# EdwardLiuyc/StaticMapping

Measured on NVIDIA H100. Metric: scan-pair alignments/sec (120k->500k pts, 30 ICP iters), higher is better.
Workload: dtype f64

## Files before the change

### include/sm_b200_debug.h

```cpp
#ifndef SM_B200_DEBUG_H_
#define SM_B200_DEBUG_H_

#include <stdint.h>

#ifdef __cplusplus
extern "C" {
#endif

int sm_debug_solve6(int device, const double* A_36, const double* b_6, double* x_6, int32_t* path);

int sm_debug_solve6_host(const double* A_36, const double* b_6, double* x_6, int32_t* path);

typedef int (*sm_debug_fdf)(const double* x_6, double* f, double* g_6, void* user);
int sm_debug_bfgs_minimize(sm_debug_fdf fn, void* user, double* x_6_inout, double grad_tol,
                           int32_t max_iterations, int32_t* iterations, int32_t* evaluations, int32_t* status);

int sm_debug_knn1_batched(int device, const double* target_3xn, int64_t n_target, const double* query_3xn,
                          int64_t n_query, double epsilon, int bucket_size, int32_t queries_per_cta,
                          int32_t* ids, double* dists2);

int sm_debug_ndt_host(int32_t op, const double* in, double* out);

int sm_debug_icp_host(int32_t op, const double* in, int64_t n, double* out);

typedef int (*sm_debug_ndt_eval)(const double* T_4x4, const double* p_6, double* sums_44, void* user);
int sm_debug_ndt_newton(sm_debug_ndt_eval fn, void* user, const double* guess_4x4, int32_t n_source, float resolution,
                        double step_size, double outlier_ratio, double transformation_epsilon, int32_t max_iterations,
                        double* final_4x4, int32_t* iterations, int32_t* evaluations, double* score);

typedef int (*sm_debug_gicp_correspond)(const double* transformation_4x4, const double* R_9, int32_t* m, void* user);
typedef int (*sm_debug_gicp_cost)(const double* T_4x4, double* S_13, void* user);
int sm_debug_gicp_outer(sm_debug_gicp_correspond correspond, sm_debug_gicp_cost cost, void* user,
                        const double* guess_4x4, double* final_4x4, int32_t* iterations, int32_t* bfgs_evaluations);

// ... 25 lines not shown
```

### staticmapping_b200/_lib.py

```python
from __future__ import annotations

import ctypes as C
import os

_HERE = os.path.dirname(os.path.abspath(__file__))
LIB_PATH = os.environ.get("SM_B200_LIB") or os.path.join(_HERE, "libsm_b200.so")


class AlignInfo(C.Structure):
    _fields_ = [("iterations", C.c_int32), ("status", C.c_int32), ("solve_path", C.c_int32),
                ("reserved", C.c_int32), ("kept", C.c_int64), ("limit", C.c_double),
                ("ms_upload", C.c_float), ("ms_prologue", C.c_float),
                ("ms_iterations", C.c_float), ("kernel_launches", C.c_int32),
                ("ms_knn", C.c_float), ("ms_accum", C.c_float), ("ms_finish", C.c_float),
                ("profiled_iterations", C.c_int32), ("evaluations", C.c_int32),
                ("trans_probability", C.c_double), ("mean_neighbors", C.c_double),
                ("aux", C.c_double * 4)]


class Pair(C.Structure):
    _fields_ = [("source", C.c_void_p), ("n_source", C.c_int64), ("target", C.c_void_p),
                ("target_normals", C.c_void_p), ("n_target", C.c_int64), ("guess", C.c_void_p),
                ("on_device", C.c_int32), ("reserved", C.c_int32)]

# ... 42 lines not shown
    "sm_debug_bfgs_minimize": (C.c_int, [_VP, _VP, _VP, C.c_double, C.c_int32, _VP, _VP, _VP]),
    "sm_debug_ndt_newton": (C.c_int, [_VP, _VP, _VP, C.c_int32, C.c_float, C.c_double, C.c_double, C.c_double, C.c_int32,
                                      _VP, _VP, _VP, _VP]),
    "sm_debug_normals_leaf": (C.c_int, [_VP, C.c_int32, _VP, _VP, _VP]),
    "sm_debug_voxel_index": (C.c_int, [C.c_int32, _VP, C.c_float, C.c_int32, _VP]),
    "sm_debug_gicp_point": (C.c_int, [C.c_int32, _VP, _VP]),
    "sm_debug_gicp_outer": (C.c_int, [_VP, _VP, _VP, _VP, _VP, _VP, _VP]),
    "sm_debug_gicp_host": (C.c_int, [C.c_int32, _VP, _VP]),
    "sm_debug_motion_host": (C.c_int, [_VP, C.c_int64, _DP, _VP]),
    "sm_debug_inner_compensation_host": (C.c_int, [_DP, _VP, _VP, _VP, C.c_int64, _VP, _VP]),
    "sm_debug_icp_host": (C.c_int, [C.c_int32, _VP, C.c_int64, _VP]),
    "sm_debug_ndt_leaf": (C.c_int, [_VP, C.c_int32, C.c_int32, C.c_double, _VP, _VP, _VP, _VP, _VP]),
    "sm_debug_ndt_term": (C.c_int, [_VP, C.c_double, C.c_float, C.c_int32, _VP, _VP, _VP, _VP, _VP]),
    "sm_debug_ndt_host": (C.c_int, [C.c_int32, _VP, _VP]),
    "sm_debug_knn1_batched": (C.c_int, [C.c_int, _VP, C.c_int64, _VP, C.c_int64, C.c_double, C.c_int, C.c_int32, _VP, _VP]),
    "sm_device_count": (C.c_int, []),
    "sm_version": (C.c_char_p, []),
}


def lib():
    global _lib
    if _lib is None:
        if not os.path.exists(LIB_PATH):
            raise RuntimeError(
                f"{LIB_PATH} not found: build it with `python -c 'import __graft_entry__ as g; "
                "g.build()'` (nvcc, sm_90a).  staticmapping_b200 has no CPU fallback.")
        _lib = C.CDLL(LIB_PATH)
        for name, (res, args) in SIGNATURES.items():
            fn = getattr(_lib, name)
# ... 4 lines not shown
```

### staticmapping_b200/csrc/icp.cu

```cuda
#include "common.cuh"
#include "kernels.h"
#include "icp_dev.cuh"
#include "knn_smem.cuh"
#include "linalg_dev.cuh"
#include "motion_dev.cuh"

#include <nvtx3/nvToolsExt.h>

namespace smb {
using namespace dev;
namespace {

__global__ void __launch_bounds__(256)
mean_partial_kernel(const double* __restrict__ raw, int64_t stride, int n,
                    double* __restrict__ partials) {
  __shared__ double sm[3][8];
  double s[3] = {0.0, 0.0, 0.0};
  const int base = blockIdx.x * 1024;
  for (int r = 0; r < 4; ++r) {
    const int i = base + r * 256 + threadIdx.x;
    if (i < n) { s[0] += raw[i]; s[1] += raw[stride + i]; s[2] += raw[2 * stride + i]; }
  }
  for (int d = 0; d < 3; ++d) {
    double v = s[d];
// ... 49 lines not shown
  st->hist_len = 1; st->iteration = 0; st->done = 0; st->status = 0; st->solve_path = 0;
  st->final_score = 0.0; st->limit = 0.0; st->kept = 0;
}

__device__ __forceinline__ uint32_t spread10(uint32_t v) {
  v &= 1023u;
  v = (v | (v << 16)) & 0x030000ffu;
  v = (v | (v << 8)) & 0x0300f00fu;
  v = (v | (v << 4)) & 0x030c30c3u;
  v = (v | (v << 2)) & 0x09249249u;
  return v;
}

__global__ void apply_g0_kernel(const double* __restrict__ in, double* __restrict__ out,
                                int64_t stride, int n, const IcpState* __restrict__ st,
                                uint64_t* __restrict__ keys, uint32_t* __restrict__ vals) {
  const int i = blockIdx.x * blockDim.x + threadIdx.x;
  if (i >= n) return;
  double px, py, pz;
  transform_point(st->G0, in[i], in[stride + i], in[2 * stride + i], px, py, pz);
  out[i] = px; out[stride + i] = py; out[2 * stride + i] = pz;
  const uint32_t ix = (uint32_t)(int)floor(px * 4.0), iy = (uint32_t)(int)floor(py * 4.0),
                 iz = (uint32_t)(int)floor(pz * 4.0);
  keys[i] = (uint64_t)(spread10(ix) | (spread10(iy) << 1) | (spread10(iz) << 2));
  vals[i] = (uint32_t)i;
}

__global__ void gather_source_kernel(const double* __restrict__ in, double* __restrict__ out,
                                     int64_t stride, int n, const uint32_t* __restrict__ perm) {
  const int i = blockIdx.x * blockDim.x + threadIdx.x;
  if (i >= n) return;
  const uint32_t s = perm[i];
  out[i] = in[s]; out[stride + i] = in[stride + s]; out[2 * stride + i] = in[2 * stride + s];
// ... 16 lines not shown
__global__ void __launch_bounds__(kKnnCtaThreads, SMB_KNN_MIN_CTAS)
icp_knn_kernel(IcpBuffers b, IcpParams p, int per_cta, const double* __restrict__ deskewed) {
  extern __shared__ __align__(128) unsigned char knn_smem[];
  if (b.state->done) return;
  uint64_t* bar; double* T;
  const SmemTree tree = stage_tree(b.kc, knn_smem, &bar, &T);
  if (threadIdx.x < 16) T[threadIdx.x] = b.state->T_iter[threadIdx.x];
  __syncthreads();
  const int begin = blockIdx.x * per_cta, end = min(begin + per_cta, p.n_source);
  int i = begin + threadIdx.x;
  double px = 0.0, py = 0.0, pz = 0.0;
  if (i < end) load_query<kComp>(b, T, deskewed, i, px, py, pz);
  mbar_wait(bar, 0);
  while (i < end) {
    int slot; double d2;
    knn1_smem<kAllSmem>(tree, px, py, pz, p.max_error2, slot, d2);
    b.slot[i] = slot;
    b.d2[i] = d2;
    if (finite_d2(d2)) atomicAdd(&b.hist[dist_bin(d2)], 1u);
    i += kKnnCtaThreads;
    if (i < end) load_query<kComp>(b, T, deskewed, i, px, py, pz);
  }
}

template <bool kAllSmem, bool kComp>
__global__ void __launch_bounds__(kKnnCtaThreads, SMB_KNN_MIN_CTAS)
icp_knn_batch_kernel(IcpBuffers b, IcpParams p, int per_cta, const double* __restrict__ deskewed) {
  extern __shared__ __align__(128) unsigned char knn_smem[];
  if (b.state->done) return;
  uint64_t* bar; double* T;
  const SmemTree tree = stage_tree(b.kc, knn_smem, &bar, &T);
  if (threadIdx.x < 16) T[threadIdx.x] = b.state->T_iter[threadIdx.x];
  __syncthreads();
  const int begin = blockIdx.x * per_cta, end = min(begin + per_cta, p.n_source);
  mbar_wait(bar, 0);
  knn_batch_cta<kAllSmem>(
      tree, begin, end, per_cta, p.max_error2, b.knn_items,
      [&](int i, double& x, double& y, double& z) { load_query<kComp>(b, T, deskewed, i, x, y, z); },
      [&](int i, int best, double head) { b.slot[i] = best; b.d2[i] = head; },
      [&](int i, double& head, int& best) { head = __ldcg(b.d2 + i); best = __ldcg(b.slot + i); },
      [&](int i, int slot, double d2) {
        b.slot[i] = slot;
        b.d2[i] = d2;
        if (finite_d2(d2)) atomicAdd(&b.hist[dist_bin(d2)], 1u);
      });
}

template <bool kComp>
__global__ void __launch_bounds__(kAccThreads)
icp_accum_kernel(IcpBuffers b, IcpParams p, const double* __restrict__ deskewed) {
  __shared__ uint32_t warp_tot[8];
  __shared__ BinSel sel_sm;
// ... 74 lines not shown
      const int64_t dst = tile0 + off + __popc(m[r] & ((1u << lane) - 1u));
      b.cand_key[dst] = (unsigned long long)__double_as_longlong(d2[r]);
      double2* o = reinterpret_cast<double2*>(b.cand_terms + 8 * dst);
      o[0] = make_double2(F[r][0], F[r][1]); o[1] = make_double2(F[r][2], F[r][3]);
      o[2] = make_double2(F[r][4], F[r][5]); o[3] = make_double2(dot[r], sq[r]);
    }
    base += tot;
  }
  if (threadIdx.x == 0) b.cand_cnt[blockIdx.x] = base;
  block_reduce_sums<kAccThreads>(acc, red, b.partials + (int64_t)blockIdx.x * 32);
}

template <bool kAllSmem>
__global__ void __launch_bounds__(kKnnCtaThreads)
knn_query_kernel(KdCompact kc, const double* __restrict__ query, int64_t qstride, int nq,
                 double max_error2, int per_cta, int32_t* __restrict__ ids, double* __restrict__ d2) {
  extern __shared__ __align__(128) unsigned char knn_smem[];
  uint64_t* bar; double* extra;
  const SmemTree tree = stage_tree(kc, knn_smem, &bar, &extra);
  const int begin = blockIdx.x * per_cta, end = min(begin + per_cta, nq);
  mbar_wait(bar, 0);
  for (int i = begin + threadIdx.x; i < end; i += kKnnCtaThreads) {
    int slot; double d;
    knn1_smem<kAllSmem>(tree, query[i], query[qstride + i], query[2 * qstride + i], max_error2, slot, d);
    ids[i] = slot >= 0 ? kc.pid[slot] : -1;
    d2[i] = d;
  }
}


template <bool kAllSmem>
__global__ void __launch_bounds__(kKnnCtaThreads, SMB_KNN_MIN_CTAS)
knn_query_batch_kernel(KdCompact kc, const double* __restrict__ query, int64_t qstride, int nq,
                       double max_error2, int per_cta, int32_t* __restrict__ ids, double* __restrict__ d2,
                       int4* __restrict__ items) {
  extern __shared__ __align__(128) unsigned char knn_smem[];
  uint64_t* bar; double* extra;
  const SmemTree tree = stage_tree(kc, knn_smem, &bar, &extra);
  const int begin = blockIdx.x * per_cta, end = min(begin + per_cta, nq);
  mbar_wait(bar, 0);
  knn_batch_cta<kAllSmem>(
      tree, begin, end, per_cta, max_error2, items,
      [&](int i, double& x, double& y, double& z) { x = query[i]; y = query[qstride + i]; z = query[2 * qstride + i]; },
      [&](int i, int best, double head) { ids[i] = best; d2[i] = head; },
      [&](int i, double& head, int& best) { head = __ldcg(d2 + i); best = __ldcg(ids + i); },
      [&](int i, int slot, double d) { ids[i] = slot >= 0 ? kc.pid[slot] : -1; d2[i] = d; });
}

}

int icp_accum_blocks(int n_source) { return ceil_div(n_source, kAccTile); }

static void knn_geometry(int nq, int queries_per_cta, int* grid, int* per_cta) {
  int per = queries_per_cta > 0 ? queries_per_cta : kKnnCtaThreads;
  per = ((per + kKnnCtaThreads - 1) / kKnnCtaThreads) * kKnnCtaThreads;
  *per_cta = per;
  *grid = ceil_div(nq, per);
}

int knn_query(const KdCompact& kc, const double* query, int64_t qstride, int nq, double max_error2,
              int32_t* ids, double* d2, cudaStream_t stream, int queries_per_cta, int4* items) {
  if (nq <= 0) return 0;
  int grid, per;
  knn_geometry(nq, queries_per_cta, &grid, &per);
  const size_t smem = knn_smem_bytes(kc.levels);
  const bool all = kc.levels <= kKnnSmemLevels;
  if (per > kKnnCtaThreads) {
    if (!items) return -1;
    if (all) knn_query_batch_kernel<true><<<grid, kKnnCtaThreads, smem, stream>>>(kc, query, qstride, nq, max_error2, per, ids, d2, items);
    else knn_query_batch_kernel<false><<<grid, kKnnCtaThreads, smem, stream>>>(kc, query, qstride, nq, max_error2, per, ids, d2, items);
  } else if (all) {
    knn_query_kernel<true><<<grid, kKnnCtaThreads, smem, stream>>>(kc, query, qstride, nq, max_error2, per, ids, d2);
  } else {
    knn_query_kernel<false><<<grid, kKnnCtaThreads, smem, stream>>>(kc, query, qstride, nq, max_error2, per, ids, d2);
  }
  SMB_CUDA_OK(cudaGetLastError());
  return 0;
}

int icp_prologue(const IcpBuffers& b, const IcpParams& p, const double* guess_dev,
                 KdWorkspace& ws, const KdCompactTree& tree, cudaStream_t stream) {
  const int nt = p.n_target, ns = p.n_source;
  const int nparts = ceil_div(nt, 1024);
  mean_partial_kernel<<<nparts, 256, 0, stream>>>(b.tgt_raw, b.tstride, nt, b.mean_partials);
  center_kernel<<<ceil_div(nt, 256), 256, 0, stream>>>(b.tgt_raw, b.tgt, b.tstride, nt,
                                                      b.mean_partials, nparts, b.state);
  nvtxRangePushA("BuildKdTree");
  int rc = tree.build(b.tgt, b.nrm, b.tstride, nt, 8, ws, stream);
  nvtxRangePop();
  if (rc) return rc;
  const RadixPairs& sp = b.src_sort;
  icp_init_kernel<<<1, 256, 0, stream>>>(b.state, guess_dev, b.hist);
  apply_g0_kernel<<<ceil_div(ns, 256), 256, 0, stream>>>(b.src_raw, b.src_g0, b.sstride, ns, b.state,
                                                        sp.keys[0], sp.vals[0]);
  rc = radix_sort_pairs_u64(sp.keys[0], sp.vals[0], sp.keys[1], sp.vals[1], ns, 1, b.sstride, sp.scratch, stream, 4);
  if (rc) return rc;
  gather_source_kernel<<<ceil_div(ns, 256), 256, 0, stream>>>(b.src_g0, b.src0, b.sstride, ns, sp.vals[0]);
  SMB_CUDA_OK(cudaGetLastError());
  return 0;
}

template <bool kComp>
void icp_enqueue_search(const IcpBuffers& b, const IcpParams& p, int grid, int per, size_t smem, cudaStream_t stream,
                        const double* deskewed) {
  if (per > kKnnCtaThreads) {
    if (p.tree_levels <= kKnnSmemLevels)
      icp_knn_batch_kernel<true, kComp><<<grid, kKnnCtaThreads, smem, stream>>>(b, p, per, deskewed);
    else
      icp_knn_batch_kernel<false, kComp><<<grid, kKnnCtaThreads, smem, stream>>>(b, p, per, deskewed);
// ... 45 lines not shown
```

### staticmapping_b200/csrc/kernels.h

```cpp
#ifndef SM_B200_KERNELS_H_
#define SM_B200_KERNELS_H_

#include <cuda_runtime.h>
#include <stdint.h>

#include <utility>

#include "common.cuh"

namespace smb {

struct DevBuf {
  void* p = nullptr;
  size_t cap = 0;
  DevBuf() = default;
  DevBuf(DevBuf&& o) noexcept : p(o.p), cap(o.cap) { o.p = nullptr; o.cap = 0; }
  DevBuf& operator=(DevBuf&& o) noexcept { std::swap(p, o.p); std::swap(cap, o.cap); return *this; }
  ~DevBuf() { if (p) cudaFree(p); }
  int reserve(size_t bytes) {
    if (bytes <= cap) return 0;
    if (p) { SMB_CUDA_OK(cudaFree(p)); p = nullptr; cap = 0; }
    const size_t want = bytes + bytes / 8 + 4096;
    SMB_CUDA_OK(cudaMalloc(&p, want));
    cap = want;
// ... 93 lines not shown
struct IcpBuffers {
  double* tgt;
  double* tgt_raw;
  double* nrm;
  int64_t tstride;
  KdNode* nodes;
  uint32_t* leaf_order;
  KdCompact kc;
  double* src_raw;
  double* src_g0;
  double* src0;
  RadixPairs src_sort;
  int64_t sstride;
  int32_t* slot;
  int4* knn_items;
  double* d2;
  uint32_t* hist;
  uint32_t* hist2;
  double* sums;
  double* cand_terms;
  unsigned long long* cand_key;
  uint32_t* cand_cnt;
  double* partials;
  double* mean_partials;
  IcpState* state;
};

int icp_accum_blocks(int n_source);
int icp_prologue(const IcpBuffers& b, const IcpParams& p, const double* guess_dev,
                 KdWorkspace& ws, const KdCompactTree& tree, cudaStream_t stream);
int icp_enqueue_iterations(const IcpBuffers& b, const IcpParams& p, int start_iteration, int count,
                           cudaStream_t stream, cudaEvent_t* events, double* deskewed = nullptr);
void icp_finish_launch(const IcpBuffers& b, const IcpParams& p, int nblocks_b, cudaStream_t stream);
int knn_query(const KdCompact& kc, const double* query, int64_t qstride, int nq, double max_error2,
              int32_t* ids, double* d2, cudaStream_t stream, int queries_per_cta = 0, int4* items = nullptr);

void icp_deskew_launch(const IcpBuffers& b, const IcpParams& p, double* out, cudaStream_t stream);

struct NdtGrid {
  float inv_leaf;
  int min_b[3], div_b[3], mul[3];
  int n_voxels;
};
struct NdtLeaf {
  double mean[3];
  double icov[9];
  float centroid[3];
  int nr_points;
  int searchable;
  int pad;
// ... 88 lines not shown
```

### staticmapping_b200/csrc/knn_smem.cuh

```cuda
#ifndef SM_B200_KNN_SMEM_CUH_
#define SM_B200_KNN_SMEM_CUH_

#include "common.cuh"
#include "kernels.h"

namespace smb {
namespace dev {

#ifndef SMB_KNN_THREADS
#define SMB_KNN_THREADS 256
#endif
#ifndef SMB_KNN_SMEM_LEVELS
#define SMB_KNN_SMEM_LEVELS 11
#endif
#ifndef SMB_KNN_HALF_SCAN
#define SMB_KNN_HALF_SCAN 1
#endif
#ifndef SMB_KNN_Q_FROM_SMEM
#define SMB_KNN_Q_FROM_SMEM 0
#endif
#if SMB_KNN_Q_FROM_SMEM
#define SMB_KNN_Q(t, reg, d) ((t).sq[(d) * kKnnCtaThreads])
#else
#define SMB_KNN_Q(t, reg, d) (reg)
#endif
constexpr int kKnnCtaThreads = SMB_KNN_THREADS;
constexpr int kKnnSmemLevels = SMB_KNN_SMEM_LEVELS;
constexpr int kKnnCtasPerSm = 1024 / kKnnCtaThreads;

struct SmemTree {
  const double* s_cut;
// ... 189 lines not shown
    ldg_node(t.g_node, h, cut, cd);
    if (cd == 3) break;
    const double q = t.sq[cd * kKnnCtaThreads];
    const double old_off = t.sq[(3 + cd) * kKnnCtaThreads];
    const double new_off = dsub(q, cut);
    const double rd_new = dadd(rd, dadd(-dmul(old_off, old_off), dmul(new_off, new_off)));
    const int right = q > cut ? 1 : 0;
    if (dmul(rd_new, me2) < head) pending |= 1u << l;
    h = 2 * h + 1 + right;
    ++l;
  }
  hp1 = h + 1; ll = l;
  return (h + 1 - (1 << l)) << (t.levels - l);
}

template <bool kAllSmem>
__device__ __forceinline__ void knn_root_visit(const SmemTree& t, double qx, double qy, double qz, double me2,
                                               double& head, int& best, int& hp1_out, int& ll_out, uint32_t& mask_out) {
  head = __longlong_as_double(0x7ff0000000000000ll);
  best = -1;
  t.sq[0] = qx; t.sq[kKnnCtaThreads] = qy; t.sq[2 * kKnnCtaThreads] = qz;
  const int lsm = kAllSmem ? t.levels : min(t.levels, kKnnSmemLevels);
  int h = 0, l = 0;
  bool leaf = false;
  while (l < lsm) {
    const int cd = t.s_dim[h];
    if (cd == 3) { leaf = true; break; }
    h = 2 * h + 1 + (t.sq[cd * kKnnCtaThreads] > t.s_cut[h] ? 1 : 0);
    ++l;
  }
  if (!kAllSmem && !leaf) {
    while (l < t.levels) {
      double cut; int cd;
      ldg_node(t.g_node, h, cut, cd);
      if (cd == 3) break;
      h = 2 * h + 1 + (t.sq[cd * kKnnCtaThreads] > cut ? 1 : 0);
      ++l;
    }
  }
  scan_bucket(t.pb, (h + 1 - (1 << l)) << (t.levels - l), qx, qy, qz, head, best);
  const int hp1 = h + 1, ll = l;
  uint32_t mask = 0u;
  for (int a = 0; a < ll; ++a) {
    double cut; int cd;
    path_node(t, (hp1 >> (ll - a)) - 1, cut, cd);
    const double off = dsub(t.sq[cd * kKnnCtaThreads], cut);
    if (dmul(dmul(off, off), me2) < head) mask |= 1u << a;
  }
  hp1_out = hp1; ll_out = ll; mask_out = mask;
}

template <bool kAllSmem>
__device__ __forceinline__ void knn1_smem(const SmemTree& t, double qx, double qy, double qz, double me2,
                                          int& best_out, double& d2_out) {
  double head, rd; int best, hp1, ll, h; uint32_t pending, turns = 0u;
  knn_root_visit<kAllSmem>(t, qx, qy, qz, me2, head, best, hp1, ll, pending);
  while (knn_pop(t, me2, head, hp1, ll, pending, turns, h, rd)) {
    const int bucket = knn_descend(t, me2, head, h, rd, pending, hp1, ll);
    scan_bucket(t.pb, bucket, SMB_KNN_Q(t, qx, 0), SMB_KNN_Q(t, qy, 1), SMB_KNN_Q(t, qz, 2), head, best);
  }
  best_out = best;
  d2_out = head;
}

struct KnnItem { int i, hp1, ll; uint32_t mask; };

template <typename LoadQuery, typename StoreResult>
__device__ __forceinline__ void knn_far_phase(const SmemTree& t, double me2, const int4* __restrict__ items,
                                              int n_items, LoadQuery load_query, StoreResult store_result) {
  const unsigned lt = (1u << (threadIdx.x & 31)) - 1u;
  int next = 0;
// ... 19 lines not shown
    double rd = 0.0;
    if (qi >= 0) {
      go = knn_pop(t, me2, head, hp1, ll, pending, turns, h, rd);
      if (!go) { store_result(qi, best, head); qi = -1; }
    }
    if (go) {
      const int bucket = knn_descend(t, me2, head, h, rd, pending, hp1, ll);
      scan_bucket(t.pb, bucket, t.sq[0], t.sq[kKnnCtaThreads], t.sq[2 * kKnnCtaThreads], head, best);
    }
  }
}

constexpr int kKnnMaxQpt = 4;
template <bool kAllSmem, typename LoadQ, typename Park, typename Unpark, typename Finish>
__device__ __forceinline__ void knn_batch_cta(const SmemTree& tree, int begin, int end, int per_cta, double me2,
                                              int4* __restrict__ items_all, LoadQ load_q, Park park,
                                              Unpark unpark, Finish finish) {
  const int warp = threadIdx.x >> 5;
  const unsigned lt = (1u << (threadIdx.x & 31)) - 1u;
  for (int base = begin, qb; base < end; base += kKnnCtaThreads * qb) {
    qb = min(kKnnMaxQpt, (begin + per_cta - base) / kKnnCtaThreads);
    int4* items = items_all + base + warp * 32 * qb;
    int count = 0;
    for (int j = 0; j < qb; ++j) {
      const int i = base + j * kKnnCtaThreads + threadIdx.x;
      bool far = false;
      int4 item = make_int4(0, 0, 0, 0);
      if (i < end) {
        double px, py, pz, head;
        int best, hp1, ll;
        uint32_t mask;
        load_q(i, px, py, pz);
        knn_root_visit<kAllSmem>(tree, px, py, pz, me2, head, best, hp1, ll, mask);
        if (mask == 0u) {
          finish(i, best, head);
        } else {
          park(i, best, head);
          far = true;
          item = make_int4(i, hp1, ll, (int)mask);
        }
      }
      const unsigned m = __ballot_sync(0xffffffffu, far);
      if (far) items[count + __popc(m & lt)] = item;
      count += __popc(m);
    }
    __syncwarp();
    knn_far_phase(tree, me2, items, count,
                  [&](int i, double& qx, double& qy, double& qz, double& head, int& best) {
// ... 13 lines not shown
```

### staticmapping_b200/csrc/sm_api.cu

```cuda
#include "../../include/sm_b200.h"
#include "../../include/sm_b200_debug.h"

#include <math.h>
#include <stdlib.h>
#include <string.h>

#include <atomic>
#include <iterator>
#include <mutex>
#include <string>
#include <thread>
#include <vector>

#include <nvtx3/nvToolsExt.h>

#include "common.cuh"
#include "icp_dev.cuh"
#include "kernels.h"
#include "linalg_dev.cuh"
#include "gicp_host.h"
#include "ndt_host.h"

namespace smb {

// ... 415 lines not shown
  {
    const float q = h->icp.dist_outlier_ratio;
    if (!(q >= 0.0f && q <= 1.0f)) return fail(h, SM_ERR_BAD_ARGUMENT, "Align: dist_outlier_ratio outside [0, 1] (icp_fast.cc:68)");
    if (!(h->icp.knn_epsilon >= 0.0f)) return fail(h, SM_ERR_BAD_ARGUMENT, "Align: knn_epsilon must be >= 0");
  }
  NvtxRange nvtx_align("IcpFast::Align");
  const int ns = (int)h->n_source, nt = (int)h->n_target;
  const int levels = kd_num_levels(nt, 8);
  const int nb = icp_accum_blocks(ns);
  H_RC(f.tgt.reserve((size_t)(3 * f.tstride) * sizeof(double)));
  H_RC(f.src0.reserve((size_t)(3 * f.sstride) * sizeof(double)));
  H_RC(f.src_g0.reserve((size_t)(3 * f.sstride) * sizeof(double)));
  H_RC(f.src_sort.reserve(RadixPairs::bytes(f.sstride, ns)));
  H_RC(f.tree.reserve(nt, 8, KdCompactTree::kNormals));
  const size_t slot_bytes = (((size_t)ns * sizeof(int32_t) + 64 + 255) / 256) * 256;
  H_RC(f.slot.reserve(slot_bytes + ((size_t)ns + kKnnItemSlack) * sizeof(int4)));
  H_RC(f.d2.reserve((size_t)ns * sizeof(double)));
  H_RC(f.hist.reserve((2 * kHistBins + 64) * sizeof(uint32_t) + 32 * sizeof(double)));
  H_RC(f.cand_terms.reserve((size_t)nb * 512 * 8 * sizeof(double)));
  H_RC(f.cand_key.reserve((size_t)nb * 512 * sizeof(unsigned long long)));
  H_RC(f.cand_cnt.reserve((size_t)nb * sizeof(uint32_t)));
  H_RC(f.partials.reserve((size_t)nb * 32 * sizeof(double)));
  H_RC(f.mean_partials.reserve((size_t)ceil_div(nt, 1024) * 4 * sizeof(double)));
  H_RC(f.state.reserve(sizeof(IcpState)));
  H_RC(f.guess.reserve(16 * sizeof(double)));
  KdWorkspace& ws = r.ws;
  H_RC(ws.carve(h->kdws, nt, 8));

  IcpBuffers& b = r.b;
  b.tgt = (double*)f.tgt.p; b.tgt_raw = (double*)f.tgt_raw.p; b.nrm = (double*)f.nrm.p;
  b.tstride = f.tstride;
  b.nodes = (KdNode*)f.tree.nodes.p; b.leaf_order = (uint32_t*)f.tree.leaf_order.p;
  b.kc = f.tree.view();
  b.src_raw = (double*)f.src_raw.p; b.src0 = (double*)f.src0.p; b.sstride = f.sstride;
  b.src_g0 = (double*)f.src_g0.p;
  b.src_sort.carve(f.src_sort.p, f.sstride);
  b.slot = (int32_t*)f.slot.p;
  b.knn_items = reinterpret_cast<int4*>((char*)f.slot.p + slot_bytes);
  b.d2 = (double*)f.d2.p; b.hist = (uint32_t*)f.hist.p;
  b.hist2 = b.hist + kHistBins;
  b.sums = (double*)(b.hist + 2 * kHistBins + 64);
  b.cand_terms = (double*)f.cand_terms.p;
  b.cand_key = (unsigned long long*)f.cand_key.p; b.cand_cnt = (uint32_t*)f.cand_cnt.p;
  b.partials = (double*)f.partials.p; b.mean_partials = (double*)f.mean_partials.p;
  b.state = (IcpState*)f.state.p;
  IcpParams& p = r.p;
  p.n_source = ns; p.n_target = nt;
  p.max_iteration = h->icp.max_iteration;
  p.dist_outlier_ratio = h->icp.dist_outlier_ratio;
  const double eps = (double)h->icp.knn_epsilon;
  p.max_error2 = (1.0 + eps) * (1.0 + eps);
  p.disable_convergence = h->icp.disable_convergence_check ? 1 : 0;
  p.knn_queries_per_cta = h->icp.knn_queries_per_cta;
// ... 885 lines not shown
  DevBuf stage;
  SMB_RC(np.reserve((int)n));
  SMB_RC(upload_soa(points, n, false, stage, np.input(), np.stride, s));
  uint32_t m = 0;
  SMB_RC(np.run((int)n, s, &m));
  if (m > 0) {
    SMB_CUDA_OK(cudaMemcpyAsync(out_points, np.points(), (size_t)3 * m * sizeof(double), cudaMemcpyDeviceToHost, s));
    SMB_CUDA_OK(cudaMemcpyAsync(out_normals, np.normals(), (size_t)3 * m * sizeof(double), cudaMemcpyDeviceToHost, s));
    SMB_CUDA_OK(cudaStreamSynchronize(s));
  }
  *m_out = (int64_t)m;
  return SM_OK;
}

static int knn1_impl(int device, const double* target, int64_t nt, const double* query, int64_t nq,
                     double epsilon, int bucket, int queries_per_cta, int32_t* ids, double* d2);

int sm_knn1(int device, const double* target, int64_t nt, const double* query, int64_t nq,
            double epsilon, int bucket, int32_t* ids, double* d2) {
  return knn1_impl(device, target, nt, query, nq, epsilon, bucket, 0, ids, d2);
}

int sm_debug_knn1_batched(int device, const double* target, int64_t nt, const double* query, int64_t nq,
                          double epsilon, int bucket, int32_t queries_per_cta, int32_t* ids, double* d2) {
  if (queries_per_cta < 0 || queries_per_cta > (1 << 20)) return SM_ERR_BAD_ARGUMENT;
  return knn1_impl(device, target, nt, query, nq, epsilon, bucket, queries_per_cta, ids, d2);
}

static int knn1_impl(int device, const double* target, int64_t nt, const double* query, int64_t nq,
                     double epsilon, int bucket, int queries_per_cta, int32_t* ids, double* d2) {
  if (!target || !query || nt <= 0 || nt > (1 << 30) || nq < 0 || nq > (1 << 30) || bucket < 2 || bucket > 8 ||
      !(epsilon >= 0.0))
    return SM_ERR_BAD_ARGUMENT;
  int ndev = 0;
  if (cudaGetDeviceCount(&ndev) != cudaSuccess || ndev <= 0) return SM_ERR_NO_DEVICE;
  SMB_CUDA_OK(cudaSetDevice(device));
  cudaStream_t s = nullptr;
  const int64_t ts = pad64(nt), qs = pad64(nq > 0 ? nq : 1);
  const int levels = kd_num_levels((int)nt, bucket);
  if (levels > 24) return SM_ERR_BAD_ARGUMENT;
  DevBuf stage, tgt, qry, kdws, ids_d, d2_d, items;
  KdCompactTree tree;
  SMB_RC(stage.reserve((size_t)3 * (size_t)(nt > nq ? nt : nq) * sizeof(double)));
  SMB_RC(tgt.reserve((size_t)3 * ts * sizeof(double)));
  SMB_RC(qry.reserve((size_t)3 * qs * sizeof(double)));
  SMB_RC(tree.reserve((int)nt, bucket, KdCompactTree::kIds));
  KdWorkspace ws;
  SMB_RC(ws.carve(kdws, (int)nt, bucket));
  SMB_RC(ids_d.reserve((size_t)(nq > 0 ? nq : 1) * sizeof(int32_t)));
  SMB_RC(d2_d.reserve((size_t)(nq > 0 ? nq : 1) * sizeof(double)));
  SMB_RC(items.reserve(((size_t)nq + kKnnItemSlack) * sizeof(int4)));
  SMB_RC(upload_soa(target, nt, false, stage, (double*)tgt.p, ts, s));
  SMB_CUDA_OK(cudaStreamSynchronize(s));
  SMB_RC(tree.build((const double*)tgt.p, nullptr, ts, (int)nt, bucket, ws, s));
  if (nq > 0) {
    SMB_RC(upload_soa(query, nq, false, stage, (double*)qry.p, qs, s));
    SMB_RC(knn_query(tree.view(), (const double*)qry.p, qs, (int)nq, (1.0 + epsilon) * (1.0 + epsilon), (int32_t*)ids_d.p,
                     (double*)d2_d.p, s, queries_per_cta, (int4*)items.p));
    SMB_CUDA_OK(cudaMemcpyAsync(ids, ids_d.p, (size_t)nq * sizeof(int32_t), cudaMemcpyDeviceToHost, s));
    SMB_CUDA_OK(cudaMemcpyAsync(d2, d2_d.p, (size_t)nq * sizeof(double), cudaMemcpyDeviceToHost, s));
  }
  SMB_CUDA_OK(cudaStreamSynchronize(s));
  return SM_OK;
}

}
```

### staticmapping_b200/registrators.py

```python
from __future__ import annotations

import ctypes as C
import enum
import xml.etree.ElementTree as ET
from dataclasses import dataclass, field
from typing import Optional

import numpy as np

from . import _lib


class Type(enum.IntEnum):
    kNoType = 0
    kIcpPM = 1
    kLibicp = 2
    kNdtWithGicp = 3
    kLegoLoam = 4
    kNdt = 5
    kFastIcp = 6


class CheckFailure(RuntimeError):
    """Raised where the reference would glog CHECK-fail (abort)."""
# ... 331 lines not shown
    ids = np.empty(q.shape[0], dtype=np.int32)
    d2 = np.empty(q.shape[0], dtype=np.float64)
    if queries_per_cta:
        rc = lib.sm_debug_knn1_batched(device, t.ctypes.data, t.shape[0], q.ctypes.data, q.shape[0], float(epsilon),
                                       int(bucket_size), int(queries_per_cta), ids.ctypes.data, d2.ctypes.data)
    else:
        rc = lib.sm_knn1(device, t.ctypes.data, t.shape[0], q.ctypes.data, q.shape[0], float(epsilon),
                         int(bucket_size), ids.ctypes.data, d2.ctypes.data)
    if rc == -20:
        raise RuntimeError("staticmapping_b200: no CUDA device (no CPU fallback)")
    if rc != 0:
        raise RuntimeError(f"sm_knn1 failed with {rc}")
    return ids, d2


def CalculateNormals(points, device=0) -> EigenCloud:
    lib = _lib.lib()
    p = np.ascontiguousarray(np.asarray(points, dtype=np.float64))
    out_p = np.empty_like(p)
    out_n = np.empty_like(p)
    m = C.c_int64(0)
    rc = lib.sm_calculate_normals(device, p.ctypes.data, p.shape[0], out_p.ctypes.data,
                                  out_n.ctypes.data, C.byref(m))
    if rc == -20:
        raise RuntimeError("staticmapping_b200: no CUDA device (no CPU fallback)")
    if rc != 0:
        raise RuntimeError(f"sm_calculate_normals failed with {rc}")
    return EigenCloud(out_p[:m.value].copy(), out_n[:m.value].copy())


# ... 114 lines not shown
```

Before: 763.5.

## Warm-start ICP kd-tree nearest-neighbour search from previous iteration's leaf hint

Stores each source point's kd-tree leaf from the previous ICP iteration and, on the next query, checks the stored path bit by bit against the current query, skipping the root descent down to the first level that no longer matches. It also prefetches the hinted leaf bucket into L1 and disables the half-scan option. This aims to cut descent cost in the KNN kernel, since points move little between iterations. In exchange it adds a per-point hint buffer read and write, a full-depth unrolled validation loop, and extra global loads for deep trees.

Measured after the change: 762.9 (median of 6 runs). About the same (-0.1%).

```diff
diff --git a/include/sm_b200_debug.h b/include/sm_b200_debug.h
--- a/include/sm_b200_debug.h
+++ b/include/sm_b200_debug.h
@@ -18,6 +18,10 @@
 int sm_debug_knn1_batched(int device, const double* target_3xn, int64_t n_target, const double* query_3xn,
                           int64_t n_query, double epsilon, int bucket_size, int32_t queries_per_cta,
                           int32_t* ids, double* dists2);
+
+int sm_debug_knn1_hinted(int device, const double* target_3xn, int64_t n_target, const double* query_3xn,
+                         int64_t n_query, double epsilon, int bucket_size, int32_t queries_per_cta,
+                         const int32_t* hints_in, int32_t* ids, double* dists2, int32_t* hints_out);
 
 int sm_debug_ndt_host(int32_t op, const double* in, double* out);
 
diff --git a/profiles/knn_leaf_hints.py b/profiles/knn_leaf_hints.py
--- /dev/null
+++ b/profiles/knn_leaf_hints.py
@@ -0,0 +1,98 @@
+#!/usr/bin/env python
+import argparse
+import os
+import runpy
+import sys
+import time
+
+import numpy as np
+
+ROOT = os.path.dirname(os.path.dirname(os.path.abspath(__file__)))
+sys.path.insert(0, ROOT)
+sys.path.insert(0, os.path.join(ROOT, "tests"))
+
+
+def tree_arrays(model):
+    size = 1 << (model.levels + 1)
+    cut = np.zeros(size)
+    dim = np.full(size, 4, dtype=np.int8)
+    for h, d in model.dim.items():
+        dim[h] = d
+    for h, c in model.cut.items():
+        cut[h] = c
+    return cut, dim
+
+
+def descend_all(cut, dim, levels, Q):
+    h = np.zeros(len(Q), dtype=np.int64)
+    done = np.zeros(len(Q), dtype=bool)
+    rows = np.arange(len(Q))
+    for _ in range(levels):
+        d = dim[h]
+        done |= d == 3
+        if done.all():
+            break
+        cd = np.where(done, 0, d)
+        right = (Q[rows, cd] > cut[h]).astype(np.int64)
+        h = np.where(done, h, 2 * h + 1 + right)
+    return h + 1
+
+
+def first_mismatch_level(prev, cur):
+    lp = np.floor(np.log2(prev)).astype(np.int64)
+    lc = np.floor(np.log2(cur)).astype(np.int64)
+    lm = np.minimum(lp, lc)
+    a, b = prev >> (lp - lm), cur >> (lc - lm)
+    x = a ^ b
+    diff = np.where(x > 0, np.floor(np.log2(np.maximum(x, 1))).astype(np.int64) + 1, 0)
+    return lm - diff
+
+
+def cpu_part():
+    import bench
+    import oracle_lib as O
+    from gpu_knn_hint_model import GpuKnnHintModel
+
+    src, sub, _ = bench.make_workload(0)
+    t0 = time.time()
+    tp, tn = O.calculate_normals(sub)
+    out = O.icp_fast_align(src, tp, tn, max_iteration=bench.ITERATIONS, disable_convergence_check=True, trace=True)
+    mean = tp.sum(axis=0) / tp.shape[0]
+    model = GpuKnnHintModel(tp - mean)
+    cut, dim = tree_arrays(model)
+    print(f"pair 0: {src.shape[0]} queries, {tp.shape[0]} target points, tree of {model.levels} levels "
+          f"(oracle and model tree in {time.time() - t0:.0f} s)")
+    S0 = src - mean
+    Ts = [np.eye(4)] + [t["T_iter"] for t in out["trace"]]
+    prev = None
+    print(f"{'iter':>4} {'hit rate':>9} {'mean first-mismatch level (misses)':>36}")
+    rates = []
+    for k in range(len(out["trace"])):
+        T = Ts[k]
+        leaves = descend_all(cut, dim, model.levels, S0 @ T[:3, :3].T + T[:3, 3])
+        if prev is None:
+            print(f"{k:4d} {'-':>9} {'- (no hint yet)':>36}")
+        else:
+            hit = leaves == prev
+            miss_lv = first_mismatch_level(prev[~hit], leaves[~hit])
+            rates.append(hit.mean())
+            print(f"{k:4d} {100 * hit.mean():8.2f}% {miss_lv.mean() if len(miss_lv) else float('nan'):36.2f}")
+        prev = leaves
+    print(f"mean hit rate over iterations 1..{len(rates)}: {100 * np.mean(rates):.2f}%")
+
+
+def main():
+    ap = argparse.ArgumentParser()
+    ap.add_argument("--gpu", action="store_true", help="also the per-kernel time in bench.py's 16-in-flight regime")
+    ap.add_argument("--no-cpu", action="store_true")
+    ap.add_argument("--steps", type=int, default=5)
+    args = ap.parse_args()
+    if not args.no_cpu:
+        cpu_part()
+    if args.gpu:
+        sys.argv = [sys.argv[0], "--steps", str(args.steps)]
+        runpy.run_path(os.path.join(ROOT, "profiles", "kernel_shares.py"), run_name="__main__")
+
+
+if __name__ == "__main__":
+    main()
diff --git a/staticmapping_b200/_lib.py b/staticmapping_b200/_lib.py
--- a/staticmapping_b200/_lib.py
+++ b/staticmapping_b200/_lib.py
@@ -80,6 +80,8 @@
     "sm_debug_ndt_term": (C.c_int, [_VP, C.c_double, C.c_float, C.c_int32, _VP, _VP, _VP, _VP, _VP]),
     "sm_debug_ndt_host": (C.c_int, [C.c_int32, _VP, _VP]),
     "sm_debug_knn1_batched": (C.c_int, [C.c_int, _VP, C.c_int64, _VP, C.c_int64, C.c_double, C.c_int, C.c_int32, _VP, _VP]),
+    "sm_debug_knn1_hinted": (C.c_int, [C.c_int, _VP, C.c_int64, _VP, C.c_int64, C.c_double, C.c_int, C.c_int32, _VP, _VP,
+                                       _VP, _VP]),
     "sm_device_count": (C.c_int, []),
     "sm_version": (C.c_char_p, []),
 }
diff --git a/staticmapping_b200/csrc/icp.cu b/staticmapping_b200/csrc/icp.cu
--- a/staticmapping_b200/csrc/icp.cu
+++ b/staticmapping_b200/csrc/icp.cu
@@ -87,9 +87,11 @@
 
 __global__ void apply_g0_kernel(const double* __restrict__ in, double* __restrict__ out,
                                 int64_t stride, int n, const IcpState* __restrict__ st,
-                                uint64_t* __restrict__ keys, uint32_t* __restrict__ vals) {
+                                uint64_t* __restrict__ keys, uint32_t* __restrict__ vals,
+                                int32_t* __restrict__ leaf_hint) {
   const int i = blockIdx.x * blockDim.x + threadIdx.x;
   if (i >= n) return;
+  leaf_hint[i] = 0;
   double px, py, pz;
   transform_point(st->G0, in[i], in[stride + i], in[2 * stride + i], px, py, pz);
   out[i] = px; out[stride + i] = py; out[2 * stride + i] = pz;
@@ -136,7 +138,10 @@
   mbar_wait(bar, 0);
   while (i < end) {
     int slot; double d2;
-    knn1_smem<kAllSmem>(tree, px, py, pz, p.max_error2, slot, d2);
+    const int hint = b.leaf_hint[i];
+    int leaf = hint;
+    knn1_smem<kAllSmem>(tree, px, py, pz, p.max_error2, leaf, slot, d2);
+    if (leaf != hint) b.leaf_hint[i] = leaf;
     b.slot[i] = slot;
     b.d2[i] = d2;
     if (finite_d2(d2)) atomicAdd(&b.hist[dist_bin(d2)], 1u);
@@ -157,7 +162,7 @@
   const int begin = blockIdx.x * per_cta, end = min(begin + per_cta, p.n_source);
   mbar_wait(bar, 0);
   knn_batch_cta<kAllSmem>(
-      tree, begin, end, per_cta, p.max_error2, b.knn_items,
+      tree, begin, end, per_cta, p.max_error2, b.knn_items, b.leaf_hint,
       [&](int i, double& x, double& y, double& z) { load_query<kComp>(b, T, deskewed, i, x, y, z); },
       [&](int i, int best, double head) { b.slot[i] = best; b.d2[i] = head; },
       [&](int i, double& head, int& best) { head = __ldcg(b.d2 + i); best = __ldcg(b.slot + i); },
@@ -262,7 +267,8 @@
 template <bool kAllSmem>
 __global__ void __launch_bounds__(kKnnCtaThreads)
 knn_query_kernel(KdCompact kc, const double* __restrict__ query, int64_t qstride, int nq,
-                 double max_error2, int per_cta, int32_t* __restrict__ ids, double* __restrict__ d2) {
+                 double max_error2, int per_cta, int32_t* __restrict__ ids, double* __restrict__ d2,
+                 int32_t* __restrict__ hints) {
   extern __shared__ __align__(128) unsigned char knn_smem[];
   uint64_t* bar; double* extra;
   const SmemTree tree = stage_tree(kc, knn_smem, &bar, &extra);
@@ -270,7 +276,9 @@
   mbar_wait(bar, 0);
   for (int i = begin + threadIdx.x; i < end; i += kKnnCtaThreads) {
     int slot; double d;
-    knn1_smem<kAllSmem>(tree, query[i], query[qstride + i], query[2 * qstride + i], max_error2, slot, d);
+    int leaf = hints ? hints[i] : 0;
+    knn1_smem<kAllSmem>(tree, query[i], query[qstride + i], query[2 * qstride + i], max_error2, leaf, slot, d);
+    if (hints) hints[i] = leaf;
     ids[i] = slot >= 0 ? kc.pid[slot] : -1;
     d2[i] = d;
   }
@@ -281,14 +289,14 @@
 __global__ void __launch_bounds__(kKnnCtaThreads, SMB_KNN_MIN_CTAS)
 knn_query_batch_kernel(KdCompact kc, const double* __restrict__ query, int64_t qstride, int nq,
                        double max_error2, int per_cta, int32_t* __restrict__ ids, double* __restrict__ d2,
-                       int4* __restrict__ items) {
+                       int4* __restrict__ items, int32_t* __restrict__ hints) {
   extern __shared__ __align__(128) unsigned char knn_smem[];
   uint64_t* bar; double* extra;
   const SmemTree tree = stage_tree(kc, knn_smem, &bar, &extra);
   const int begin = blockIdx.x * per_cta, end = min(begin + per_cta, nq);
   mbar_wait(bar, 0);
   knn_batch_cta<kAllSmem>(
-      tree, begin, end, per_cta, max_error2, items,
+      tree, begin, end, per_cta, max_error2, items, hints,
       [&](int i, double& x, double& y, double& z) { x = query[i]; y = query[qstride + i]; z = query[2 * qstride + i]; },
       [&](int i, int best, double head) { ids[i] = best; d2[i] = head; },
       [&](int i, double& head, int& best) { head = __ldcg(d2 + i); best = __ldcg(ids + i); },
@@ -307,7 +315,7 @@
 }
 
 int knn_query(const KdCompact& kc, const double* query, int64_t qstride, int nq, double max_error2,
-              int32_t* ids, double* d2, cudaStream_t stream, int queries_per_cta, int4* items) {
+              int32_t* ids, double* d2, cudaStream_t stream, int queries_per_cta, int4* items, int32_t* hints) {
   if (nq <= 0) return 0;
   int grid, per;
   knn_geometry(nq, queries_per_cta, &grid, &per);
@@ -315,12 +323,12 @@
   const bool all = kc.levels <= kKnnSmemLevels;
   if (per > kKnnCtaThreads) {
     if (!items) return -1;
-    if (all) knn_query_batch_kernel<true><<<grid, kKnnCtaThreads, smem, stream>>>(kc, query, qstride, nq, max_error2, per, ids, d2, items);
-    else knn_query_batch_kernel<false><<<grid, kKnnCtaThreads, smem, stream>>>(kc, query, qstride, nq, max_error2, per, ids, d2, items);
+    if (all) knn_query_batch_kernel<true><<<grid, kKnnCtaThreads, smem, stream>>>(kc, query, qstride, nq, max_error2, per, ids, d2, items, hints);
+    else knn_query_batch_kernel<false><<<grid, kKnnCtaThreads, smem, stream>>>(kc, query, qstride, nq, max_error2, per, ids, d2, items, hints);
   } else if (all) {
-    knn_query_kernel<true><<<grid, kKnnCtaThreads, smem, stream>>>(kc, query, qstride, nq, max_error2, per, ids, d2);
+    knn_query_kernel<true><<<grid, kKnnCtaThreads, smem, stream>>>(kc, query, qstride, nq, max_error2, per, ids, d2, hints);
   } else {
-    knn_query_kernel<false><<<grid, kKnnCtaThreads, smem, stream>>>(kc, query, qstride, nq, max_error2, per, ids, d2);
+    knn_query_kernel<false><<<grid, kKnnCtaThreads, smem, stream>>>(kc, query, qstride, nq, max_error2, per, ids, d2, hints);
   }
   SMB_CUDA_OK(cudaGetLastError());
   return 0;
@@ -340,7 +348,7 @@
   const RadixPairs& sp = b.src_sort;
   icp_init_kernel<<<1, 256, 0, stream>>>(b.state, guess_dev, b.hist);
   apply_g0_kernel<<<ceil_div(ns, 256), 256, 0, stream>>>(b.src_raw, b.src_g0, b.sstride, ns, b.state,
-                                                        sp.keys[0], sp.vals[0]);
+                                                        sp.keys[0], sp.vals[0], b.leaf_hint);
   rc = radix_sort_pairs_u64(sp.keys[0], sp.vals[0], sp.keys[1], sp.vals[1], ns, 1, b.sstride, sp.scratch, stream, 4);
   if (rc) return rc;
   gather_source_kernel<<<ceil_div(ns, 256), 256, 0, stream>>>(b.src_g0, b.src0, b.sstride, ns, sp.vals[0]);
diff --git a/staticmapping_b200/csrc/kernels.h b/staticmapping_b200/csrc/kernels.h
--- a/staticmapping_b200/csrc/kernels.h
+++ b/staticmapping_b200/csrc/kernels.h
@@ -131,6 +131,7 @@
   int64_t sstride;
   int32_t* slot;
   int4* knn_items;
+  int32_t* leaf_hint;
   double* d2;
   uint32_t* hist;
   uint32_t* hist2;
@@ -150,7 +151,8 @@
                            cudaStream_t stream, cudaEvent_t* events, double* deskewed = nullptr);
 void icp_finish_launch(const IcpBuffers& b, const IcpParams& p, int nblocks_b, cudaStream_t stream);
 int knn_query(const KdCompact& kc, const double* query, int64_t qstride, int nq, double max_error2,
-              int32_t* ids, double* d2, cudaStream_t stream, int queries_per_cta = 0, int4* items = nullptr);
+              int32_t* ids, double* d2, cudaStream_t stream, int queries_per_cta = 0, int4* items = nullptr,
+              int32_t* hints = nullptr);
 
 void icp_deskew_launch(const IcpBuffers& b, const IcpParams& p, double* out, cudaStream_t stream);
 
diff --git a/staticmapping_b200/csrc/knn_smem.cuh b/staticmapping_b200/csrc/knn_smem.cuh
--- a/staticmapping_b200/csrc/knn_smem.cuh
+++ b/staticmapping_b200/csrc/knn_smem.cuh
@@ -14,7 +14,7 @@
 #define SMB_KNN_SMEM_LEVELS 11
 #endif
 #ifndef SMB_KNN_HALF_SCAN
-#define SMB_KNN_HALF_SCAN 1
+#define SMB_KNN_HALF_SCAN 0
 #endif
 #ifndef SMB_KNN_Q_FROM_SMEM
 #define SMB_KNN_Q_FROM_SMEM 0
@@ -234,8 +234,50 @@
   return (h + 1 - (1 << l)) << (t.levels - l);
 }
 
+__device__ __forceinline__ void prefetch_l1(const void* p) {
+  asm volatile("prefetch.global.L1 [%0];" ::"l"(__cvta_generic_to_global(p)));
+}
+
+constexpr int kKnnHintLdgLevels = 4;
+
+__device__ __forceinline__ uint32_t hint_level_bad(const SmemTree& t, int hint, int hl, int a, double cut, int cd) {
+  const bool right = ((hint >> (a < hl ? hl - a - 1 : 0)) & 1) != 0;
+  const bool bad = (cd == 3) | ((t.sq[cd * kKnnCtaThreads] > cut) != right);
+  return bad && a < hl ? 1u << a : 0u;
+}
+
 template <bool kAllSmem>
-__device__ __forceinline__ void knn_root_visit(const SmemTree& t, double qx, double qy, double qz, double me2,
+__device__ __forceinline__ int knn_hint_check(const SmemTree& t, int hint, int hl) {
+  uint32_t bad = 0u;
+#pragma unroll
+  for (int a = 0; a < kKnnSmemLevels; ++a) {
+    const int n = a < hl ? (hint >> (hl - a)) - 1 : 0;
+    bad |= hint_level_bad(t, hint, hl, a, t.s_cut[n], t.s_dim[n]);
+  }
+  if (kAllSmem) {
+    const int lcd = t.s_dim[hl < t.levels ? hint - 1 : 0];
+    if (hl < t.levels && lcd != 3) bad |= 1u << hl;
+  } else {
+#pragma unroll
+    for (int a = kKnnSmemLevels; a < kKnnSmemLevels + kKnnHintLdgLevels; ++a) {
+      double cut; int cd;
+      ldg_node(t.g_node, a < hl ? (hint >> (hl - a)) - 1 : 0, cut, cd);
+      bad |= hint_level_bad(t, hint, hl, a, cut, cd);
+    }
+    double lcut; int lcd;
+    ldg_node(t.g_node, hl < t.levels ? hint - 1 : 0, lcut, lcd);
+    if (hl < t.levels && lcd != 3) bad |= 1u << hl;
+    for (int a = kKnnSmemLevels + kKnnHintLdgLevels; a < hl; ++a) {
+      double cut; int cd;
+      ldg_node(t.g_node, (hint >> (hl - a)) - 1, cut, cd);
+      bad |= hint_level_bad(t, hint, hl, a, cut, cd);
+    }
+  }
+  return bad != 0u ? __ffs(bad) - 1 : hl;
+}
+
+template <bool kAllSmem>
+__device__ __forceinline__ void knn_root_visit(const SmemTree& t, double qx, double qy, double qz, double me2, int hint,
                                                double& head, int& best, int& hp1_out, int& ll_out, uint32_t& mask_out) {
   head = __longlong_as_double(0x7ff0000000000000ll);
   best = -1;
@@ -243,7 +285,16 @@
   const int lsm = kAllSmem ? t.levels : min(t.levels, kKnnSmemLevels);
   int h = 0, l = 0;
   bool leaf = false;
-  while (l < lsm) {
+  if (hint != 0) {
+    const int hl = 31 - __clz(hint);
+    const char* pb = reinterpret_cast<const char*>(t.pb + (int64_t)((hint - (1 << hl)) << (t.levels - hl)) * 24);
+    prefetch_l1(pb);
+    prefetch_l1(pb + 191);
+    l = knn_hint_check<kAllSmem>(t, hint, hl);
+    h = (hint >> (hl - l)) - 1;
+    leaf = l == hl;
+  }
+  while (!leaf && l < lsm) {
     const int cd = t.s_dim[h];
     if (cd == 3) { leaf = true; break; }
     h = 2 * h + 1 + (t.sq[cd * kKnnCtaThreads] > t.s_cut[h] ? 1 : 0);
@@ -272,9 +323,10 @@
 
 template <bool kAllSmem>
 __device__ __forceinline__ void knn1_smem(const SmemTree& t, double qx, double qy, double qz, double me2,
-                                          int& best_out, double& d2_out) {
+                                          int& leaf, int& best_out, double& d2_out) {
   double head, rd; int best, hp1, ll, h; uint32_t pending, turns = 0u;
-  knn_root_visit<kAllSmem>(t, qx, qy, qz, me2, head, best, hp1, ll, pending);
+  knn_root_visit<kAllSmem>(t, qx, qy, qz, me2, leaf, head, best, hp1, ll, pending);
+  leaf = hp1;
   while (knn_pop(t, me2, head, hp1, ll, pending, turns, h, rd)) {
     const int bucket = knn_descend(t, me2, head, h, rd, pending, hp1, ll);
     scan_bucket(t.pb, bucket, SMB_KNN_Q(t, qx, 0), SMB_KNN_Q(t, qy, 1), SMB_KNN_Q(t, qz, 2), head, best);
@@ -324,8 +376,8 @@
 constexpr int kKnnMaxQpt = 4;
 template <bool kAllSmem, typename LoadQ, typename Park, typename Unpark, typename Finish>
 __device__ __forceinline__ void knn_batch_cta(const SmemTree& tree, int begin, int end, int per_cta, double me2,
-                                              int4* __restrict__ items_all, LoadQ load_q, Park park,
-                                              Unpark unpark, Finish finish) {
+                                              int4* __restrict__ items_all, int32_t* __restrict__ hints, LoadQ load_q,
+                                              Park park, Unpark unpark, Finish finish) {
   const int warp = threadIdx.x >> 5;
   const unsigned lt = (1u << (threadIdx.x & 31)) - 1u;
   for (int base = begin, qb; base < end; base += kKnnCtaThreads * qb) {
@@ -340,8 +392,10 @@
         double px, py, pz, head;
         int best, hp1, ll;
         uint32_t mask;
+        const int hint = hints ? hints[i] : 0;
         load_q(i, px, py, pz);
-        knn_root_visit<kAllSmem>(tree, px, py, pz, me2, head, best, hp1, ll, mask);
+        knn_root_visit<kAllSmem>(tree, px, py, pz, me2, hint, head, best, hp1, ll, mask);
+        if (hints && hp1 != hint) hints[i] = hp1;
         if (mask == 0u) {
           finish(i, best, head);
         } else {
diff --git a/staticmapping_b200/csrc/sm_api.cu b/staticmapping_b200/csrc/sm_api.cu
--- a/staticmapping_b200/csrc/sm_api.cu
+++ b/staticmapping_b200/csrc/sm_api.cu
@@ -453,7 +453,7 @@
   H_RC(f.src_sort.reserve(RadixPairs::bytes(f.sstride, ns)));
   H_RC(f.tree.reserve(nt, 8, KdCompactTree::kNormals));
   const size_t slot_bytes = (((size_t)ns * sizeof(int32_t) + 64 + 255) / 256) * 256;
-  H_RC(f.slot.reserve(slot_bytes + ((size_t)ns + kKnnItemSlack) * sizeof(int4)));
+  H_RC(f.slot.reserve(2 * slot_bytes + ((size_t)ns + kKnnItemSlack) * sizeof(int4)));
   H_RC(f.d2.reserve((size_t)ns * sizeof(double)));
   H_RC(f.hist.reserve((2 * kHistBins + 64) * sizeof(uint32_t) + 32 * sizeof(double)));
   H_RC(f.cand_terms.reserve((size_t)nb * 512 * 8 * sizeof(double)));
@@ -475,7 +475,8 @@
   b.src_g0 = (double*)f.src_g0.p;
   b.src_sort.carve(f.src_sort.p, f.sstride);
   b.slot = (int32_t*)f.slot.p;
-  b.knn_items = reinterpret_cast<int4*>((char*)f.slot.p + slot_bytes);
+  b.leaf_hint = reinterpret_cast<int32_t*>((char*)f.slot.p + slot_bytes);
+  b.knn_items = reinterpret_cast<int4*>((char*)f.slot.p + 2 * slot_bytes);
   b.d2 = (double*)f.d2.p; b.hist = (uint32_t*)f.hist.p;
   b.hist2 = b.hist + kHistBins;
   b.sums = (double*)(b.hist + 2 * kHistBins + 64);
@@ -1391,7 +1392,8 @@
 }
 
 static int knn1_impl(int device, const double* target, int64_t nt, const double* query, int64_t nq,
-                     double epsilon, int bucket, int queries_per_cta, int32_t* ids, double* d2);
+                     double epsilon, int bucket, int queries_per_cta, int32_t* ids, double* d2,
+                     const int32_t* hints_in = nullptr, int32_t* hints_out = nullptr);
 
 int sm_knn1(int device, const double* target, int64_t nt, const double* query, int64_t nq,
             double epsilon, int bucket, int32_t* ids, double* d2) {
@@ -1404,8 +1406,26 @@
   return knn1_impl(device, target, nt, query, nq, epsilon, bucket, queries_per_cta, ids, d2);
 }
 
+int sm_debug_knn1_hinted(int device, const double* target, int64_t nt, const double* query, int64_t nq,
+                         double epsilon, int bucket, int32_t queries_per_cta, const int32_t* hints_in, int32_t* ids,
+                         double* d2, int32_t* hints_out) {
+  if (queries_per_cta < 0 || queries_per_cta > (1 << 20) || (nq > 0 && (!hints_in || !hints_out)))
+    return SM_ERR_BAD_ARGUMENT;
+  return knn1_impl(device, target, nt, query, nq, epsilon, bucket, queries_per_cta, ids, d2, hints_in, hints_out);
+}
+
+static bool is_leaf_hp1(const std::vector<uint8_t>& dim, int levels, int32_t hp1) {
+  if (hp1 <= 0) return false;
+  const int hl = 31 - __builtin_clz((unsigned)hp1);
+  if (hl > levels) return false;
+  for (int a = 0; a < hl; ++a)
+    if (dim[(hp1 >> (hl - a)) - 1] == 3) return false;
+  return hl == levels || dim[hp1 - 1] == 3;
+}
+
 static int knn1_impl(int device, const double* target, int64_t nt, const double* query, int64_t nq,
-                     double epsilon, int bucket, int queries_per_cta, int32_t* ids, double* d2) {
+                     double epsilon, int bucket, int queries_per_cta, int32_t* ids, double* d2,
+                     const int32_t* hints_in, int32_t* hints_out) {
   if (!target || !query || nt <= 0 || nt > (1 << 30) || nq < 0 || nq > (1 << 30) || bucket < 2 || bucket > 8 ||
       !(epsilon >= 0.0))
     return SM_ERR_BAD_ARGUMENT;
@@ -1416,7 +1436,7 @@
   const int64_t ts = pad64(nt), qs = pad64(nq > 0 ? nq : 1);
   const int levels = kd_num_levels((int)nt, bucket);
   if (levels > 24) return SM_ERR_BAD_ARGUMENT;
-  DevBuf stage, tgt, qry, kdws, ids_d, d2_d, items;
+  DevBuf stage, tgt, qry, kdws, ids_d, d2_d, items, hints_d;
   KdCompactTree tree;
   SMB_RC(stage.reserve((size_t)3 * (size_t)(nt > nq ? nt : nq) * sizeof(double)));
   SMB_RC(tgt.reserve((size_t)3 * ts * sizeof(double)));
@@ -1430,12 +1450,23 @@
   SMB_RC(upload_soa(target, nt, false, stage, (double*)tgt.p, ts, s));
   SMB_CUDA_OK(cudaStreamSynchronize(s));
   SMB_RC(tree.build((const double*)tgt.p, nullptr, ts, (int)nt, bucket, ws, s));
+  if (hints_in && nq > 0) {
+    std::vector<uint8_t> dim((size_t)1 << levels);
+    SMB_CUDA_OK(cudaMemcpyAsync(dim.data(), tree.dim.p, dim.size(), cudaMemcpyDeviceToHost, s));
+    SMB_CUDA_OK(cudaStreamSynchronize(s));
+    for (int64_t i = 0; i < nq; ++i)
+      if (hints_in[i] != 0 && !is_leaf_hp1(dim, levels, hints_in[i])) return SM_ERR_BAD_ARGUMENT;
+    SMB_RC(hints_d.reserve((size_t)nq * sizeof(int32_t)));
+    SMB_CUDA_OK(cudaMemcpyAsync(hints_d.p, hints_in, (size_t)nq * sizeof(int32_t), cudaMemcpyHostToDevice, s));
+  }
   if (nq > 0) {
     SMB_RC(upload_soa(query, nq, false, stage, (double*)qry.p, qs, s));
     SMB_RC(knn_query(tree.view(), (const double*)qry.p, qs, (int)nq, (1.0 + epsilon) * (1.0 + epsilon), (int32_t*)ids_d.p,
-                     (double*)d2_d.p, s, queries_per_cta, (int4*)items.p));
+                     (double*)d2_d.p, s, queries_per_cta, (int4*)items.p, hints_in ? (int32_t*)hints_d.p : nullptr));
     SMB_CUDA_OK(cudaMemcpyAsync(ids, ids_d.p, (size_t)nq * sizeof(int32_t), cudaMemcpyDeviceToHost, s));
     SMB_CUDA_OK(cudaMemcpyAsync(d2, d2_d.p, (size_t)nq * sizeof(double), cudaMemcpyDeviceToHost, s));
+    if (hints_in)
+      SMB_CUDA_OK(cudaMemcpyAsync(hints_out, hints_d.p, (size_t)nq * sizeof(int32_t), cudaMemcpyDeviceToHost, s));
   }
   SMB_CUDA_OK(cudaStreamSynchronize(s));
   return SM_OK;
diff --git a/staticmapping_b200/registrators.py b/staticmapping_b200/registrators.py
--- a/staticmapping_b200/registrators.py
+++ b/staticmapping_b200/registrators.py
@@ -369,6 +369,26 @@
     return ids, d2
 
 
+def knn1_hinted(target, query, hints, epsilon=3.16, bucket_size=8, device=0, queries_per_cta=0):
+    lib = _lib.lib()
+    t = np.ascontiguousarray(np.asarray(target, dtype=np.float64))
+    q = np.ascontiguousarray(np.asarray(query, dtype=np.float64))
+    h = np.ascontiguousarray(np.asarray(hints, dtype=np.int32))
+    if h.shape != (q.shape[0],):
+        raise ValueError("one hint per query")
+    ids = np.empty(q.shape[0], dtype=np.int32)
+    d2 = np.empty(q.shape[0], dtype=np.float64)
+    leaves = np.empty(q.shape[0], dtype=np.int32)
+    rc = lib.sm_debug_knn1_hinted(device, t.ctypes.data, t.shape[0], q.ctypes.data, q.shape[0], float(epsilon),
+                                  int(bucket_size), int(queries_per_cta), h.ctypes.data, ids.ctypes.data,
+                                  d2.ctypes.data, leaves.ctypes.data)
+    if rc == -20:
+        raise RuntimeError("staticmapping_b200: no CUDA device (no CPU fallback)")
+    if rc != 0:
+        raise RuntimeError(f"sm_debug_knn1_hinted failed with {rc}")
+    return ids, d2, leaves
+
+
 def CalculateNormals(points, device=0) -> EigenCloud:
     lib = _lib.lib()
     p = np.ascontiguousarray(np.asarray(points, dtype=np.float64))
```
